# Aster32/GAN-DANet

Measured on AMD Instinct MI355X. Metric: train samples/sec (G+D step) on 256x256 tiles, higher is better.
Workload: dtype bf16; 1 GPU; full G+D train step, 8ch 256x256 -> 1024x1024 tiles, batch 32/GPU (global 32), perceptual=on, SSIM evaluated, AdamW x2; survey_config=3, per_gpu_batch=32, global_batch=32, tile=256, parallelism=dp1

## Files before the change

### gan-danet_amd/csrc/conv3x3.hip

```cpp
#include "common.h"
#include "tile_mma.h"
#include "../../include/gandanet.h"

namespace {

using gd::acc_row;
using gd::bf16x8_native_t;
typedef unsigned int u32x4_t __attribute__((ext_vector_type(4)));

constexpr int TW = 32;
constexpr int PW = TW + 2;
constexpr int CK = 32;
constexpr int LD = CK + 8;

__global__ void pack_w_kernel(const float* __restrict__ a, long a_sm, long a_sc, long a_st, int M, int Ck, int flip,
                              int BM, int nchunks, unsigned short* __restrict__ wp, long total) {
    for (long i = (long)blockIdx.x * blockDim.x + threadIdx.x; i < total; i += (long)gridDim.x * blockDim.x) {
        const int cc = (int)(i % CK);
        long t = i / CK;
        const int mm = (int)(t % BM);
        t /= BM;
        const int tap = (int)(t % 9);
        t /= 9;
        const int chunk = (int)(t % nchunks);
        const int mt = (int)(t / nchunks);
        const int m = mt * BM + mm, c = chunk * CK + cc;
        float v = 0.f;
        if (m < M && c < Ck) v = a[(long)m * a_sm + (long)c * a_sc + (long)(flip ? 8 - tap : tap) * a_st];
        wp[i] = gd_f2bf(v);
    }
}

template <int BM, int TH, int S>
__global__ __launch_bounds__(256, 2) void conv3x3_halo_kernel(const gd_conv_desc d, const unsigned short* __restrict__ wp,
                                                             int tiles_x, int nchunks) {
    constexpr int WAVES_M = 2, WAVES_N = 2;
    constexpr int TM = BM / (32 * WAVES_M);
    constexpr int TN = TH / WAVES_N;
    constexpr int PH = S * (TH - 1) + 3;
    constexpr int PWk = S * (TW - 1) + 3;
    constexpr int NPIX = PH * PWk;
    constexpr int WCHUNKS = 3 * BM * CK / 8;
    constexpr int WPT = WCHUNKS / 256;
    static_assert(WCHUNKS % 256 == 0, "weight stage must divide evenly");

    __shared__ __attribute__((aligned(16))) unsigned short patch[NPIX * LD];
    __shared__ __attribute__((aligned(16))) unsigned short wts[3 * BM * LD];

    const int tid = threadIdx.x, lane = tid & 63, wave = tid >> 6;
    const int r = lane & 31, h = lane >> 5;
    const int wm = wave >> 1, wn = wave & 1;
    const int b = blockIdx.z;
    const int mt = blockIdx.y;
    const int ty = blockIdx.x / tiles_x, tx = blockIdx.x - ty * tiles_x;
    const int y0 = ty * TH, x0 = tx * TW;
    const int H = d.Hi, W = d.Wi;
    const int Ho = d.Ho, Wo = d.Wo;
    const long HW = (long)H * W, HWo = (long)Ho * Wo;
    const float* ximg = d.x + (long)b * d.x_bs;

    f32x16_t acc[TM][TN];
#pragma unroll
    for (int i = 0; i < TM; ++i)
#pragma unroll
        for (int j = 0; j < TN; ++j)
#pragma unroll
            for (int e = 0; e < 16; ++e) acc[i][j][e] = 0.f;

    const unsigned short* wbase = wp + (long)mt * nchunks * 9 * BM * CK;
    u32x4_t wreg[WPT];
    auto load_w = [&](int chunk, int ky) {
        const u32x4_t* src = reinterpret_cast<const u32x4_t*>(wbase + ((long)chunk * 9 + ky * 3) * BM * CK);
#pragma unroll
        for (int i = 0; i < WPT; ++i) wreg[i] = src[tid + i * 256];
    };
    auto store_w = [&]() {
#pragma unroll
        for (int i = 0; i < WPT; ++i) {
            const int v = tid + i * 256;
            const int row = v >> 2, q = v & 3;
            *reinterpret_cast<u32x4_t*>(wts + row * LD + q * 8) = wreg[i];
        }
    };

    for (int chunk = 0; chunk < nchunks; ++chunk) {
        const int c0 = chunk * CK;
        load_w(chunk, 0);
        for (int w = tid; w < 2 * NPIX; w += 256) {
            const int half = w >= NPIX ? 1 : 0;
            const int pix = w - half * NPIX;
            const int py = pix / PWk, px = pix - py * PWk;
            const int iy = S * y0 - 1 + py, ix = S * x0 - 1 + px;
            const bool inside = iy >= 0 && iy < H && ix >= 0 && ix < W;
            const int cb = c0 + half * 16;
            const float* p = ximg + (long)cb * HW + (long)iy * W + ix;
            unsigned int* dst = reinterpret_cast<unsigned int*>(patch + pix * LD + half * 16);
#pragma unroll
            for (int j = 0; j < 8; ++j) {
                const int c = cb + 2 * j;
                float v0 = 0.f, v1 = 0.f;
                if (inside) {
                    if (c < d.Ck) v0 = p[(long)(2 * j) * HW];
                    if (c + 1 < d.Ck) v1 = p[(long)(2 * j + 1) * HW];
                    if (d.in_scale) {
                        if (c < d.Ck) {
                            v0 = fmaf(v0, d.in_scale[c], d.in_shift[c]);
                            if (d.in_relu) v0 = fmaxf(v0, 0.f);
                        }
                        if (c + 1 < d.Ck) {
                            v1 = fmaf(v1, d.in_scale[c + 1], d.in_shift[c + 1]);
                            if (d.in_relu) v1 = fmaxf(v1, 0.f);
                        }
                    }
                }
                dst[j] = gd_pack_bf2(v0, v1);
            }
        }
        for (int ky = 0; ky < 3; ++ky) {
            store_w();
            __syncthreads();
            if (ky < 2) load_w(chunk, ky + 1);
#pragma unroll
            for (int kx = 0; kx < 3; ++kx) {
#pragma unroll
                for (int ks = 0; ks < CK / 16; ++ks) {
                    bf16x8_t fa[TM], fb[TN];
#pragma unroll
                    for (int i = 0; i < TM; ++i)
                        fa[i] = *reinterpret_cast<const bf16x8_t*>(wts + (kx * BM + wm * TM * 32 + i * 32 + r) * LD +
                                                                  ks * 16 + 8 * h);
#pragma unroll
                    for (int j = 0; j < TN; ++j)
                        fb[j] = *reinterpret_cast<const bf16x8_t*>(patch + (((wn * TN + j) * S + ky) * PWk + r * S + kx) * LD +
                                                                  ks * 16 + 8 * h);
#pragma unroll
                    for (int i = 0; i < TM; ++i)
#pragma unroll
                        for (int j = 0; j < TN; ++j)
                            acc[i][j] = __builtin_amdgcn_mfma_f32_32x32x16_bf16(
                                __builtin_bit_cast(bf16x8_native_t, fa[i]), __builtin_bit_cast(bf16x8_native_t, fb[j]),
                                acc[i][j], 0, 0, 0);
                }
            }
            __syncthreads();
        }
    }

    const float alpha = d.alpha ? *d.alpha : 1.f;
    const int ox = x0 + r;
    if (ox < Wo) {
#pragma unroll
        for (int j = 0; j < TN; ++j) {
            const int oy = y0 + wn * TN + j;
            if (oy >= Ho) continue;
            const long pn = (long)oy * Wo + ox;
#pragma unroll
            for (int i = 0; i < TM; ++i)
#pragma unroll
                for (int e = 0; e < 16; ++e) {
                    const int m = mt * BM + wm * TM * 32 + i * 32 + acc_row(e, h);
                    if (m >= d.M) continue;
                    float v = acc[i][j][e] * alpha;
                    if (d.bias) v += d.bias[m];
                    if (d.res) v += d.res[(long)b * d.res_bs + (long)m * HWo + pn];
                    if (d.act == GD_ACT_RELU) v = fmaxf(v, 0.f);
                    else if (d.act == GD_ACT_LEAKY02) v = v >= 0.f ? v : 0.2f * v;
                    float* yp = reinterpret_cast<float*>(d.y) + (long)b * d.y_bs + (long)m * HWo + pn;
                    if (d.accumulate) v += *yp;
                    *yp = v;
                }
        }
    }
}

}

static inline int pick_bm(int M, int Ck) {
    if (Ck <= CK && M > 64) return 128;
    return (M <= 64 || (M % 128 != 0 && M % 128 <= 64)) ? 64 : 128;
}

extern "C" size_t gd_conv3x3_ws_bytes(int M, int Ck) {
    const int bm = pick_bm(M, Ck);
    const long mtiles = (M + bm - 1) / bm, nchunks = (Ck + CK - 1) / CK;
    return (size_t)(mtiles * bm * nchunks * CK * 9 * 2);
}

extern "C" int gd_conv3x3_eligible(const gd_conv_desc* d) {
    if (!(d && d->ks == 3 && d->pad == 1 && d->out_layout == 0 && !d->out_bf16 && d->precision == GD_PREC_BF16 &&
          d->a_bs == 0 && (d->Mstore == 0 || d->Mstore == d->M) && d->sub_step <= 1))
        return 0;
    if (d->stride == 1) return d->Hi == d->Ho && d->Wi == d->Wo;
    return d->stride == 2 && !d->transposed && (d->Hi - 1) / 2 + 1 == d->Ho && (d->Wi - 1) / 2 + 1 == d->Wo;
}

extern "C" int gd_conv3x3(const gd_conv_desc* dp, void* ws, size_t ws_bytes, void* stream) {
    GD_CHECK_ARG(dp && ws, "gd_conv3x3: null argument");
    GD_CHECK_ARG(gd_conv3x3_eligible(dp), "gd_conv3x3: descriptor not eligible (needs 3x3, pad 1, stride 1 or forward stride 2, bf16, fp32 NCHW out)");
    const gd_conv_desc& d = *dp;
    GD_CHECK_ARG(d.B > 0 && d.B <= 65535 && d.M > 0 && d.Ck > 0 && d.Hi > 0 && d.Wi > 0, "gd_conv3x3: bad sizes");
    GD_CHECK_ARG(d.a && d.x && d.y, "gd_conv3x3: null tensor");
    GD_CHECK_ARG((d.in_scale == nullptr) == (d.in_shift == nullptr), "gd_conv3x3: in_scale/in_shift must come together");
    GD_CHECK_ARG(ws_bytes >= gd_conv3x3_ws_bytes(d.M, d.Ck), "gd_conv3x3: workspace too small");
    hipStream_t s = (hipStream_t)stream;
    const int bm = pick_bm(d.M, d.Ck);
    const int mtiles = (d.M + bm - 1) / bm, nchunks = (d.Ck + CK - 1) / CK;
    const long total = (long)mtiles * nchunks * 9 * bm * CK;
    {
        int blocks = (int)((total + 255) / 256);
        if (blocks > 2048) blocks = 2048;
        hipLaunchKernelGGL(pack_w_kernel, dim3(blocks), dim3(256), 0, s, d.a, d.a_sm, d.a_sc, d.a_st, d.M, d.Ck,
                           d.transposed ? 1 : 0, bm, nchunks, (unsigned short*)ws, total);
    }
    const int th = d.stride == 1 ? 8 : 4;
    const int tiles_x = (d.Wo + TW - 1) / TW, tiles_y = (d.Ho + th - 1) / th;
    GD_CHECK_ARG((long)tiles_x * tiles_y < (1L << 31), "gd_conv3x3: image too large");
    dim3 grid(tiles_x * tiles_y, mtiles, d.B);
    const unsigned short* wpk = (const unsigned short*)ws;
    if (d.stride == 1) {
        if (bm == 64) hipLaunchKernelGGL((conv3x3_halo_kernel<64, 8, 1>), grid, dim3(256), 0, s, d, wpk, tiles_x, nchunks);
        else hipLaunchKernelGGL((conv3x3_halo_kernel<128, 8, 1>), grid, dim3(256), 0, s, d, wpk, tiles_x, nchunks);
    } else {
        if (bm == 64) hipLaunchKernelGGL((conv3x3_halo_kernel<64, 4, 2>), grid, dim3(256), 0, s, d, wpk, tiles_x, nchunks);
        else hipLaunchKernelGGL((conv3x3_halo_kernel<128, 4, 2>), grid, dim3(256), 0, s, d, wpk, tiles_x, nchunks);
    }
    GD_LAUNCH_CHECK();
    return 0;
}

namespace {

struct NhwcConvArgs {
    const unsigned short* x;
    const unsigned short* wp;
    const float* bias;
    const unsigned short* mask;
    const unsigned short* res;
    unsigned short* y;
    float* y32;
    long y32_bs;
    int H, W, Ho, Wo, K, M, act, tiles_x, nchunks;
    float slope;
    int osplit;
};

template <int BM, int S, int EPI = 0>
__global__ __launch_bounds__(256, 2) void conv3x3_nhwc_kernel(const NhwcConvArgs a) {
    constexpr int TH = S == 1 ? 8 : 4;
    constexpr int WAVES_M = 2, WAVES_N = 2;
    constexpr int TM = BM / (32 * WAVES_M);
    constexpr int TN = TH / WAVES_N;
    constexpr int PH = S * (TH - 1) + 3, PWk = S * (TW - 1) + 3, NPIX = PH * PWk;
    constexpr int WCHUNKS = 3 * BM * CK / 8;
    constexpr int WPT = WCHUNKS / 256;
    constexpr int NIT = (4 * NPIX + 255) / 256;
    static_assert(WCHUNKS % 256 == 0, "weight stage must divide evenly");

    __shared__ __attribute__((aligned(16))) unsigned short patch[NPIX * LD];
    __shared__ __attribute__((aligned(16))) unsigned short wts[3 * BM * LD];

    const int tid = threadIdx.x, lane = tid & 63, wave = tid >> 6;
    const int r = lane & 31, h = lane >> 5;
    const int wm = wave >> 1, wn = wave & 1;
    const int b = blockIdx.z, mt = blockIdx.y;
    const int ty = blockIdx.x / a.tiles_x, tx = blockIdx.x - ty * a.tiles_x;
    const int y0 = ty * TH, x0 = tx * TW;
    const int H = a.H, W = a.W, K = a.K;
    const unsigned short* ximg = a.x + (long)b * H * W * K;

    f32x16_t acc[TM][TN];
#pragma unroll
    for (int i = 0; i < TM; ++i)
#pragma unroll
        for (int j = 0; j < TN; ++j)
#pragma unroll
            for (int e = 0; e < 16; ++e) acc[i][j][e] = 0.f;

    const unsigned short* wbase = a.wp + (long)mt * a.nchunks * 9 * BM * CK;
    u32x4_t wreg[WPT];
    auto load_w = [&](int chunk, int ky) {
        const u32x4_t* src = reinterpret_cast<const u32x4_t*>(wbase + ((long)chunk * 9 + ky * 3) * BM * CK);
#pragma unroll
        for (int i = 0; i < WPT; ++i) wreg[i] = src[tid + i * 256];
    };
    auto store_w = [&]() {
#pragma unroll
        for (int i = 0; i < WPT; ++i) {
            const int v = tid + i * 256;
            const int row = v >> 2, q = v & 3;
            *reinterpret_cast<u32x4_t*>(wts + row * LD + q * 8) = wreg[i];
        }
    };

    unsigned int goff[NIT], inmask = 0, slotmask = 0;
    int loff[NIT];
#pragma unroll
    for (int it = 0; it < NIT; ++it) {
        const int w = tid + it * 256;
        const int pix = w >> 2, q = w & 3;
        const int py = pix / PWk, px = pix - py * PWk;
        const int iy = S * y0 - 1 + py, ix = S * x0 - 1 + px;
        const bool slot = w < 4 * NPIX;
        const bool inside = slot && iy >= 0 && iy < H && ix >= 0 && ix < W;
        loff[it] = pix * LD + q * 8;
        goff[it] = inside ? (unsigned int)(((long)iy * W + ix) * K + q * 8) : 0u;
        inmask |= inside ? (1u << it) : 0u;
        slotmask |= slot ? (1u << it) : 0u;
    }
    u32x4_t raw[NIT];
    auto load_patch = [&](int chunk) {
        const unsigned short* base = ximg + chunk * CK;
#pragma unroll
        for (int it = 0; it < NIT; ++it) {
            const int q = (tid + it * 256) & 3;
            const u32x4_t z = {0u, 0u, 0u, 0u};
            raw[it] = (((inmask >> it) & 1u) && chunk * CK + q * 8 < K) ? *reinterpret_cast<const u32x4_t*>(base + goff[it]) : z;
        }
    };
    auto store_patch = [&]() {
#pragma unroll
        for (int it = 0; it < NIT; ++it)
            if ((slotmask >> it) & 1u) *reinterpret_cast<u32x4_t*>(patch + loff[it]) = raw[it];
    };

    load_patch(0);
    store_patch();
    for (int chunk = 0; chunk < a.nchunks; ++chunk) {
        load_w(chunk, 0);
#pragma unroll
        for (int ky = 0; ky < 3; ++ky) {
            store_w();
            __syncthreads();
            if (ky == 0 && chunk + 1 < a.nchunks) load_patch(chunk + 1);
            if (ky < 2) load_w(chunk, ky + 1);
#pragma unroll
            for (int kx = 0; kx < 3; ++kx) {
#pragma unroll
                for (int ks = 0; ks < CK / 16; ++ks) {
                    bf16x8_t fa[TM], fb[TN];
#pragma unroll
                    for (int i = 0; i < TM; ++i)
                        fa[i] = *reinterpret_cast<const bf16x8_t*>(wts + (kx * BM + wm * TM * 32 + i * 32 + r) * LD +
                                                                  ks * 16 + 8 * h);
#pragma unroll
                    for (int j = 0; j < TN; ++j)
                        fb[j] = *reinterpret_cast<const bf16x8_t*>(patch + (((wn * TN + j) * S + ky) * PWk + r * S + kx) * LD +
                                                                  ks * 16 + 8 * h);
#pragma unroll
                    for (int i = 0; i < TM; ++i)
#pragma unroll
                        for (int j = 0; j < TN; ++j)
                            acc[i][j] = __builtin_amdgcn_mfma_f32_32x32x16_bf16(
                                __builtin_bit_cast(bf16x8_native_t, fa[i]), __builtin_bit_cast(bf16x8_native_t, fb[j]),
                                acc[i][j], 0, 0, 0);
                }
            }
            __syncthreads();
        }
        if (chunk + 1 < a.nchunks) store_patch();
    }

    if constexpr (EPI == 1) {
        constexpr int SLD = LD;
        static_assert(4 * 2 * 32 * SLD <= NPIX * LD, "per-wave scratch must fit in the patch image");
        unsigned short* scr = patch + wave * (2 * 32 * SLD);
        const int RS = a.osplit ? 3 * a.M : a.M;
        const int ox = x0 + r;
#pragma unroll
        for (int j = 0; j < TN; ++j) {
            const int oy = y0 + wn * TN + j;
            if (oy >= a.Ho) continue;
            const long prow = ((long)b * a.Ho + oy) * a.Wo;
#pragma unroll
            for (int i = 0; i < TM; ++i) {
                const int mbase = mt * BM + wm * TM * 32 + i * 32;
                if (mbase >= a.M) continue;
#pragma unroll
                for (int g = 0; g < 4; ++g) {
                    const int m = mbase + 8 * g + 4 * h;
                    const bool ok = ox < a.Wo && m < a.M;
                    float v[4];
#pragma unroll
                    for (int k = 0; k < 4; ++k) {
                        v[k] = acc[i][j][4 * g + k];
                        if (a.bias && ok) v[k] += a.bias[m + k];
                        if (a.act == 1) v[k] = fmaxf(v[k], 0.f);
                        else if (a.act == 2) v[k] = v[k] > 0.f ? v[k] : v[k] * a.slope;
                    }
                    if (ok) {
                        const long pbase = (prow + ox) * RS;
                        if (a.mask) {
                            const uint2 mk = *reinterpret_cast<const uint2*>(a.mask + pbase + m);
                            if (!((mk.x & 0x7FFFu) && !(mk.x & 0x8000u))) v[0] = 0.f;
                            if (!((mk.x >> 16) & 0x7FFFu) || (mk.x >> 31)) v[1] = 0.f;
                            if (!((mk.y & 0x7FFFu) && !(mk.y & 0x8000u))) v[2] = 0.f;
                            if (!((mk.y >> 16) & 0x7FFFu) || (mk.y >> 31)) v[3] = 0.f;
                        }
                        if (a.res) {
#pragma unroll
                            for (int part = 0; part < 2; ++part) {
                                if (part && !a.osplit) break;
                                const uint2 rr = *reinterpret_cast<const uint2*>(a.res + pbase + part * a.M + m);
                                v[0] += gd_bf2f((unsigned short)(rr.x & 0xFFFFu));
                                v[1] += gd_bf2f((unsigned short)(rr.x >> 16));
                                v[2] += gd_bf2f((unsigned short)(rr.y & 0xFFFFu));
                                v[3] += gd_bf2f((unsigned short)(rr.y >> 16));
                            }
                        }
                    }
                    uint2 hi, lo = make_uint2(0u, 0u);
                    if (a.osplit) {
                        gd_split_bf2(v[0], v[1], hi.x, lo.x);
                        gd_split_bf2(v[2], v[3], hi.y, lo.y);
                        *reinterpret_cast<uint2*>(scr + 32 * SLD + r * SLD + 8 * g + 4 * h) = lo;
                    } else {
                        hi.x = gd_pack_bf2(v[0], v[1]);
                        hi.y = gd_pack_bf2(v[2], v[3]);
                    }
                    *reinterpret_cast<uint2*>(scr + r * SLD + 8 * g + 4 * h) = hi;
                }
#pragma unroll
                for (int pass = 0; pass < 2; ++pass) {
                    const int px = pass * 16 + (lane >> 2), c8 = (lane & 3) * 8;
                    const int oxp = x0 + px, m = mbase + c8;
                    if (oxp < a.Wo && m < a.M) {
                        unsigned short* dst = a.y + (prow + oxp) * RS + m;
                        const u32x4_t vh = *reinterpret_cast<const u32x4_t*>(scr + px * SLD + c8);
                        *reinterpret_cast<u32x4_t*>(dst) = vh;
                        if (a.osplit) {
                            *reinterpret_cast<u32x4_t*>(dst + a.M) = *reinterpret_cast<const u32x4_t*>(scr + 32 * SLD + px * SLD + c8);
                            *reinterpret_cast<u32x4_t*>(dst + 2 * a.M) = vh;
                        }
                    }
                }
            }
        }
        return;
    }

    const int ox = x0 + r;
    if (ox < a.Wo) {
#pragma unroll
        for (int j = 0; j < TN; ++j) {
            const int oy = y0 + wn * TN + j;
            if (oy >= a.Ho) continue;
            const long pbase = (((long)b * a.Ho + oy) * a.Wo + ox) * (a.osplit ? 3 * a.M : a.M);
#pragma unroll
            for (int i = 0; i < TM; ++i)
#pragma unroll
                for (int g = 0; g < 4; ++g) {
                    const int m = mt * BM + wm * TM * 32 + i * 32 + 8 * g + 4 * h;
                    if (m >= a.M) continue;
                    float v[4];
#pragma unroll
                    for (int k = 0; k < 4; ++k) {
                        v[k] = acc[i][j][4 * g + k];
                        if (a.bias) v[k] += a.bias[m + k];
                        if (a.act == 1) v[k] = fmaxf(v[k], 0.f);
                        else if (a.act == 2) v[k] = v[k] > 0.f ? v[k] : v[k] * a.slope;
                    }
                    if (a.mask) {
                        const uint2 mk = *reinterpret_cast<const uint2*>(a.mask + pbase + m);
                        if (!((mk.x & 0x7FFFu) && !(mk.x & 0x8000u))) v[0] = 0.f;
                        if (!((mk.x >> 16) & 0x7FFFu) || (mk.x >> 31)) v[1] = 0.f;
                        if (!((mk.y & 0x7FFFu) && !(mk.y & 0x8000u))) v[2] = 0.f;
                        if (!((mk.y >> 16) & 0x7FFFu) || (mk.y >> 31)) v[3] = 0.f;
                    }
                    if (a.res) {
#pragma unroll
                        for (int part = 0; part < 2; ++part) {
                            if (part && !a.osplit) break;
                            const uint2 rr = *reinterpret_cast<const uint2*>(a.res + pbase + part * a.M + m);
                            v[0] += gd_bf2f((unsigned short)(rr.x & 0xFFFFu));
                            v[1] += gd_bf2f((unsigned short)(rr.x >> 16));
                            v[2] += gd_bf2f((unsigned short)(rr.y & 0xFFFFu));
                            v[3] += gd_bf2f((unsigned short)(rr.y >> 16));
                        }
                    }
                    float* yp = a.y32 + (long)b * a.y32_bs + (long)m * a.Ho * a.Wo + (long)oy * a.Wo + ox;
#pragma unroll
                    for (int k = 0; k < 4; ++k) yp[(long)k * a.Ho * a.Wo] = v[k];
                }
        }
    }
}

struct NhwcDgrad2Args {
    const unsigned short* dy;
    const unsigned short* wp;
    const unsigned short* act;
    unsigned short* dx;
    int H, W, Ho, Wo, K, M, tiles_x, nchunks;
    float slope;
    int split;
};

__global__ __launch_bounds__(256, 2) void conv3x3_nhwc_dgrad2_kernel(const NhwcDgrad2Args a) {
    constexpr int BM = 64, TH = 4;
    constexpr int TN = TH / 2;
    constexpr int PH = TH + 1, PWd = TW + 1, NPIX = PH * PWd;
    constexpr int WPT = 3 * BM * CK / 8 / 256;
    constexpr int NIT = (4 * NPIX + 255) / 256;

    __shared__ __attribute__((aligned(16))) unsigned short patch[NPIX * LD];
    __shared__ __attribute__((aligned(16))) unsigned short wts[3 * BM * LD];

    const int tid = threadIdx.x, lane = tid & 63, wave = tid >> 6;
    const int r = lane & 31, h = lane >> 5;
    const int wm = wave >> 1, wn = wave & 1;
    const int b = blockIdx.z, mt = blockIdx.y;
    const int ty = blockIdx.x / a.tiles_x, tx = blockIdx.x - ty * a.tiles_x;
    const int u0 = ty * TH, v0 = tx * TW;
    const int Ho = a.Ho, Wo = a.Wo, M = a.M;
    const unsigned short* dyimg = a.dy + (long)b * Ho * Wo * M;

    f32x16_t acc[4][TN];
#pragma unroll
    for (int c = 0; c < 4; ++c)
#pragma unroll
        for (int j = 0; j < TN; ++j)
#pragma unroll
            for (int e = 0; e < 16; ++e) acc[c][j][e] = 0.f;

    const unsigned short* wbase = a.wp + (long)mt * a.nchunks * 9 * BM * CK;
    u32x4_t wreg[WPT];
    auto load_w = [&](int chunk, int ky) {
        const u32x4_t* src = reinterpret_cast<const u32x4_t*>(wbase + ((long)chunk * 9 + ky * 3) * BM * CK);
#pragma unroll
        for (int i = 0; i < WPT; ++i) wreg[i] = src[tid + i * 256];
    };
    auto store_w = [&]() {
#pragma unroll
        for (int i = 0; i < WPT; ++i) {
            const int v = tid + i * 256;
            *reinterpret_cast<u32x4_t*>(wts + (v >> 2) * LD + (v & 3) * 8) = wreg[i];
        }
    };

    unsigned int goff[NIT], inmask = 0, slotmask = 0;
    int loff[NIT];
#pragma unroll
    for (int it = 0; it < NIT; ++it) {
        const int w = tid + it * 256;
        const int pix = w >> 2, q = w & 3;
        const int py = pix / PWd, px = pix - py * PWd;
        const int iy = u0 + py, ix = v0 + px;
        const bool slot = w < 4 * NPIX;
        const bool inside = slot && iy < Ho && ix < Wo;
        loff[it] = pix * LD + q * 8;
        goff[it] = inside ? (unsigned int)(((long)iy * Wo + ix) * M + q * 8) : 0u;
        inmask |= inside ? (1u << it) : 0u;
        slotmask |= slot ? (1u << it) : 0u;
    }
    u32x4_t raw[NIT];
    auto load_patch = [&](int chunk) {
        const unsigned short* base = dyimg + chunk * CK;
#pragma unroll
        for (int it = 0; it < NIT; ++it) {
            const int q = (tid + it * 256) & 3;
            const u32x4_t z = {0u, 0u, 0u, 0u};
            raw[it] = (((inmask >> it) & 1u) && chunk * CK + q * 8 < M) ? *reinterpret_cast<const u32x4_t*>(base + goff[it]) : z;
        }
    };
    auto store_patch = [&]() {
#pragma unroll
        for (int it = 0; it < NIT; ++it)
            if ((slotmask >> it) & 1u) *reinterpret_cast<u32x4_t*>(patch + loff[it]) = raw[it];
    };

    load_patch(0);
    store_patch();
    for (int chunk = 0; chunk < a.nchunks; ++chunk) {
        load_w(chunk, 0);
#pragma unroll
        for (int ky = 0; ky < 3; ++ky) {
            store_w();
            __syncthreads();
            if (ky == 0 && chunk + 1 < a.nchunks) load_patch(chunk + 1);
            if (ky < 2) load_w(chunk, ky + 1);
            const int py = (ky + 1) & 1, oy = ky == 0 ? 1 : 0;
#pragma unroll
            for (int kx = 0; kx < 3; ++kx) {
                const int px = (kx + 1) & 1, ox = kx == 0 ? 1 : 0;
#pragma unroll
                for (int ks = 0; ks < CK / 16; ++ks) {
                    const bf16x8_t fa = *reinterpret_cast<const bf16x8_t*>(wts + (kx * BM + wm * 32 + r) * LD + ks * 16 + 8 * h);
#pragma unroll
                    for (int j = 0; j < TN; ++j) {
                        const bf16x8_t fb = *reinterpret_cast<const bf16x8_t*>(
                            patch + ((wn * TN + j + oy) * PWd + r + ox) * LD + ks * 16 + 8 * h);
                        acc[2 * py + px][j] = __builtin_amdgcn_mfma_f32_32x32x16_bf16(
                            __builtin_bit_cast(bf16x8_native_t, fa), __builtin_bit_cast(bf16x8_native_t, fb),
                            acc[2 * py + px][j], 0, 0, 0);
                    }
                }
            }
            __syncthreads();
        }
        if (chunk + 1 < a.nchunks) store_patch();
    }

#pragma unroll
    for (int c = 0; c < 4; ++c) {
        const int py = c >> 1, px = c & 1;
        const int X = 2 * (v0 + r) + px;
        if (X >= a.W) continue;
#pragma unroll
        for (int j = 0; j < TN; ++j) {
            const int Y = 2 * (u0 + wn * TN + j) + py;
            if (Y >= a.H) continue;
            const long pbase = (((long)b * a.H + Y) * a.W + X) * (a.split ? 3 * a.K : a.K);
#pragma unroll
            for (int g = 0; g < 4; ++g) {
                const int m = mt * BM + wm * 32 + 8 * g + 4 * h;
                if (m >= a.K) continue;
                float v[4];
#pragma unroll
                for (int k = 0; k < 4; ++k) v[k] = acc[c][j][4 * g + k];
                if (a.act) {
                    const uint2 mk = *reinterpret_cast<const uint2*>(a.act + pbase + m);
                    if (!((mk.x & 0x7FFFu) && !(mk.x & 0x8000u))) v[0] *= a.slope;
                    if (!((mk.x >> 16) & 0x7FFFu) || (mk.x >> 31)) v[1] *= a.slope;
                    if (!((mk.y & 0x7FFFu) && !(mk.y & 0x8000u))) v[2] *= a.slope;
                    if (!((mk.y >> 16) & 0x7FFFu) || (mk.y >> 31)) v[3] *= a.slope;
                }
                uint2 o;
                if (a.split) {
                    uint2 lo;
                    gd_split_bf2(v[0], v[1], o.x, lo.x);
                    gd_split_bf2(v[2], v[3], o.y, lo.y);
                    *reinterpret_cast<uint2*>(a.dx + pbase + a.K + m) = lo;
                    *reinterpret_cast<uint2*>(a.dx + pbase + 2 * a.K + m) = o;
                } else {
                    o.x = gd_pack_bf2(v[0], v[1]);
                    o.y = gd_pack_bf2(v[2], v[3]);
                }
                *reinterpret_cast<uint2*>(a.dx + pbase + m) = o;
            }
        }
    }
}

}

extern "C" int gd_conv3x3_nhwc_pack(const float* w, int Cout, int Cin, int transposed, void* ws, size_t ws_bytes,
                                    void* stream) {
    GD_CHECK_ARG(w && ws && Cout > 0 && Cin > 0 && transposed >= 0 && transposed <= 2, "gd_conv3x3_nhwc_pack: bad arguments");
    const int M = transposed ? Cin : Cout, K = transposed ? Cout : Cin;
    GD_CHECK_ARG(ws_bytes >= gd_conv3x3_ws_bytes(M, K), "gd_conv3x3_nhwc_pack: workspace too small");
    const int bm = transposed == 2 ? 64 : pick_bm(M, K);
    const int mtiles = (M + bm - 1) / bm, nchunks = (K + CK - 1) / CK;
    const long total = (long)mtiles * nchunks * 9 * bm * CK;
    int blocks = (int)((total + 255) / 256);
    if (blocks > 2048) blocks = 2048;
    const long sm = transposed ? 9 : (long)Cin * 9, sc = transposed ? (long)Cin * 9 : 9;
    hipLaunchKernelGGL(pack_w_kernel, dim3(blocks), dim3(256), 0, (hipStream_t)stream, w, sm, sc, 1L, M, K,
                       transposed == 1 ? 1 : 0, bm, nchunks, (unsigned short*)ws, total);
    GD_LAUNCH_CHECK();
    return 0;
}

static int nhwc_conv_launch(const void* x, const void* wpack, const float* bias, const void* mask, const void* res,
                            void* y, int B, int H, int W, int K, int M, int stride, int act, float slope, void* stream,
                            float* y32 = nullptr, long y32_bs = 0, int osplit = 0) {
    NhwcConvArgs a;
    a.y32 = y32; a.y32_bs = y32_bs; a.osplit = osplit;
    a.x = (const unsigned short*)x; a.wp = (const unsigned short*)wpack; a.bias = bias;
    a.mask = (const unsigned short*)mask; a.res = (const unsigned short*)res; a.y = (unsigned short*)y;
    a.H = H; a.W = W; a.K = K; a.M = M; a.act = act; a.slope = slope;
    a.Ho = (H - 1) / stride + 1; a.Wo = (W - 1) / stride + 1;
    const int bm = pick_bm(M, K);
    const int mtiles = (M + bm - 1) / bm;
    a.nchunks = (K + CK - 1) / CK;
    a.tiles_x = (a.Wo + TW - 1) / TW;
    const int th = stride == 1 ? 8 : 4;
    const int tiles_y = (a.Ho + th - 1) / th;
    dim3 grid(a.tiles_x * tiles_y, mtiles, B);
    hipStream_t s = (hipStream_t)stream;
    if (!a.y32) {
        if (stride == 1) {
            if (bm == 64) hipLaunchKernelGGL((conv3x3_nhwc_kernel<64, 1, 1>), grid, dim3(256), 0, s, a);
            else hipLaunchKernelGGL((conv3x3_nhwc_kernel<128, 1, 1>), grid, dim3(256), 0, s, a);
        } else {
            if (bm == 64) hipLaunchKernelGGL((conv3x3_nhwc_kernel<64, 2, 1>), grid, dim3(256), 0, s, a);
            else hipLaunchKernelGGL((conv3x3_nhwc_kernel<128, 2, 1>), grid, dim3(256), 0, s, a);
        }
    } else if (stride == 1) {
        if (bm == 64) hipLaunchKernelGGL((conv3x3_nhwc_kernel<64, 1>), grid, dim3(256), 0, s, a);
        else hipLaunchKernelGGL((conv3x3_nhwc_kernel<128, 1>), grid, dim3(256), 0, s, a);
    } else {
        if (bm == 64) hipLaunchKernelGGL((conv3x3_nhwc_kernel<64, 2>), grid, dim3(256), 0, s, a);
        else hipLaunchKernelGGL((conv3x3_nhwc_kernel<128, 2>), grid, dim3(256), 0, s, a);
    }
    GD_LAUNCH_CHECK();
    return 0;
}

extern "C" int gd_conv3x3_nhwc(const void* x, const void* wpack, const float* bias, const void* mask, const void* res,
                               void* y, int B, int H, int W, int K, int M, int relu, int split, void* stream) {
    GD_CHECK_ARG(x && wpack && y, "gd_conv3x3_nhwc: null pointer");
    GD_CHECK_ARG(B > 0 && B <= 65535 && H > 0 && W > 0 && K > 0 && M > 0 && K % 8 == 0 && M % 8 == 0,
                 "gd_conv3x3_nhwc: channel counts must be multiples of 8");
    GD_CHECK_ARG((long)H * W * K < (1L << 31) && (long)H * W * M * (split ? 3 : 1) < (1L << 31), "gd_conv3x3_nhwc: image too large");
    return nhwc_conv_launch(x, wpack, bias, mask, res, y, B, H, W, K, M, 1, relu ? 1 : 0, 0.f, stream, nullptr, 0, split ? 1 : 0);
}

extern "C" int gd_conv3x3_nhwc_f32out(const void* x, const void* wpack, const float* bias, float* y32, long y_bs, int B, int H,
                                      int W, int K, int M, int relu, void* stream) {
    GD_CHECK_ARG(x && wpack && y32, "gd_conv3x3_nhwc_f32out: null pointer");
    GD_CHECK_ARG(B > 0 && B <= 65535 && H > 0 && W > 0 && K > 0 && M > 0 && K % 8 == 0 && M % 4 == 0 && y_bs >= (long)M * H * W,
                 "gd_conv3x3_nhwc_f32out: K must be a multiple of 8, M of 4");
    GD_CHECK_ARG((long)H * W * K < (1L << 31), "gd_conv3x3_nhwc_f32out: image too large");
    return nhwc_conv_launch(x, wpack, bias, nullptr, nullptr, nullptr, B, H, W, K, M, 1, relu ? 1 : 0, 0.f, stream, y32, y_bs);
}

extern "C" int gd_conv3x3_nhwc_s2(const void* x, const void* wpack, const float* bias, void* y, int B, int H, int W, int K,
                                  int M, int act, float slope, int split, void* stream) {
    GD_CHECK_ARG(x && wpack && y, "gd_conv3x3_nhwc_s2: null pointer");
    GD_CHECK_ARG(B > 0 && B <= 65535 && H > 0 && W > 0 && K > 0 && M > 0 && K % 8 == 0 && M % 8 == 0 && act >= 0 && act <= 2,
                 "gd_conv3x3_nhwc_s2: channel counts must be multiples of 8, act in 0..2");
    GD_CHECK_ARG((long)H * W * K < (1L << 31) && (long)H * W * M * (split ? 3 : 1) < (1L << 31), "gd_conv3x3_nhwc_s2: image too large");
    return nhwc_conv_launch(x, wpack, bias, nullptr, nullptr, y, B, H, W, K, M, 2, act, slope, stream, nullptr, 0, split ? 1 : 0);
}

extern "C" int gd_conv3x3_nhwc_s2_dgrad(const void* dy, const void* wpack_t, const void* act_out, float slope, void* dx,
                                        int B, int H, int W, int K, int M, int split, void* stream) {
    GD_CHECK_ARG(dy && wpack_t && dx, "gd_conv3x3_nhwc_s2_dgrad: null pointer");
    GD_CHECK_ARG(B > 0 && B <= 65535 && H > 0 && W > 0 && K > 0 && M > 0 && K % 8 == 0 && M % 8 == 0,
                 "gd_conv3x3_nhwc_s2_dgrad: channel counts must be multiples of 8");
    GD_CHECK_ARG((long)H * W * K * (split ? 3 : 1) < (1L << 31) && (long)H * W * M < (1L << 31), "gd_conv3x3_nhwc_s2_dgrad: image too large");
    NhwcDgrad2Args a;
    a.split = split ? 1 : 0;
    a.dy = (const unsigned short*)dy; a.wp = (const unsigned short*)wpack_t; a.act = (const unsigned short*)act_out;
    a.dx = (unsigned short*)dx; a.H = H; a.W = W; a.K = K; a.M = M; a.slope = slope;
    a.Ho = (H - 1) / 2 + 1; a.Wo = (W - 1) / 2 + 1;
    a.nchunks = (M + CK - 1) / CK;
    a.tiles_x = (a.Wo + TW - 1) / TW;
    const int tiles_y = (a.Ho + 3) / 4;
    dim3 grid(a.tiles_x * tiles_y, (K + 63) / 64, B);
    hipLaunchKernelGGL(conv3x3_nhwc_dgrad2_kernel, grid, dim3(256), 0, (hipStream_t)stream, a);
    GD_LAUNCH_CHECK();
    return 0;
}

namespace {

typedef short s16x4_t __attribute__((ext_vector_type(4)));
constexpr int WTH = 4;
constexpr int WPH = WTH + 2;
constexpr int WNPIX = WPH * PW;
constexpr int DYLD = WTH * TW + 8;

struct WgradArgs {
    const unsigned short* dy16;
    const float* dy; long dy_bs;
    const float* x; long x_bs;
    const unsigned short* x16; int x16_ld;
    const float* in_scale; const float* in_shift; int in_relu;
    float* dw;
    float* part;
    int B, M, Ck, H, W, Ho, Wo;
    int tiles_x, tiles_y, tiles_per_split;
};
typedef float f32x4u_t __attribute__((ext_vector_type(4), aligned(4)));

__device__ __forceinline__ s16x4_t lds_tr_read(const unsigned short* p) {
    return __builtin_amdgcn_ds_read_tr16_b64_v4i16((__attribute__((address_space(3))) s16x4_t*)p);
}

#ifndef GD_WGRAD_PIPED_MINW
#define GD_WGRAD_PIPED_MINW 1
#endif
template <int NW, int S, bool CS, bool PIPED = false, bool ORD = false>
__global__ __launch_bounds__(NW * 64, PIPED ? GD_WGRAD_PIPED_MINW : 2) void conv3x3_wgrad_kernel(const WgradArgs a) {
    constexpr int BM = CS ? 32 : 32 * NW, NT = 64 * NW, NCH = CS ? NW : 1;
    constexpr int PHk = S * (WTH - 1) + 3, PWk = S * (TW - 1) + 3, NPIXk = PHk * PWk;
    __shared__ __attribute__((aligned(16))) unsigned short dys[BM * DYLD];
    __shared__ __attribute__((aligned(16))) unsigned short patch[NCH * NPIXk * LD];

    const int tid = threadIdx.x, lane = tid & 63, wave = tid >> 6;
    const int r = lane & 31, h = lane >> 5;
    const int c0 = blockIdx.x * CK * NCH;
    const int m0 = blockIdx.y * BM;
    const long HW = (long)a.H * a.W;
    const long HWo = (long)a.Ho * a.Wo;
    const int ntiles = a.B * a.tiles_y * a.tiles_x;
    const int t_begin = blockIdx.z * a.tiles_per_split;
    const int t_end = min(ntiles, t_begin + a.tiles_per_split);

    f32x16_t acc[9];
#pragma unroll
    for (int t = 0; t < 9; ++t)
#pragma unroll
        for (int e = 0; e < 16; ++e) acc[t][e] = 0.f;

    const int li = lane & 15, tq = li >> 2, tp = li & 3, tg = (lane >> 4) & 1;
    const bool vec_ok = (a.Wo % 4) == 0;

    constexpr bool piped = PIPED;
    constexpr int NDY = PIPED ? (BM * 32 + NT - 1) / NT : 1;
    constexpr int NXI = PIPED ? (4 * NCH * NPIXk + NT - 1) / NT : 1;
    uint2 rdy[NDY];
    u32x4_t rxp[NXI];
    auto load_regs = [&](int t) {
        const int b = t / (a.tiles_y * a.tiles_x);
        const int rem = t - b * (a.tiles_y * a.tiles_x);
        const int ty_ = rem / a.tiles_x, tx_ = rem - ty_ * a.tiles_x;
        const int y0 = ty_ * WTH, x0 = tx_ * TW;
#pragma unroll
        for (int k = 0; k < NDY; ++k) {
            const int idx = tid + k * NT;
            const int m = idx >> 5, v = idx & 31;
            const int yy = y0 + (v >> 3), xx = x0 + (v & 7) * 4;
            uint2 w = make_uint2(0u, 0u);
            if (idx < BM * 32 && m0 + m < a.M && yy < a.Ho) {
                const unsigned short* p = a.dy16 + ((long)b * a.M + m0 + m) * HWo + (long)yy * a.Wo + xx;
                if (vec_ok && xx + 3 < a.Wo) {
                    w = *reinterpret_cast<const uint2*>(p);
                } else {
                    unsigned int e0 = xx + 0 < a.Wo ? p[0] : 0u, e1 = xx + 1 < a.Wo ? p[1] : 0u;
                    unsigned int e2 = xx + 2 < a.Wo ? p[2] : 0u, e3 = xx + 3 < a.Wo ? p[3] : 0u;
                    w.x = e0 | (e1 << 16);
                    w.y = e2 | (e3 << 16);
                }
            }
            rdy[k] = w;
        }
#pragma unroll
        for (int k = 0; k < NXI; ++k) {
            const int w = tid + k * NT;
            const int oc = w / NPIXk;
            const int q = oc & 3, chk = oc >> 2;
            const int pix = w - oc * NPIXk;
            const int py = pix / PWk, px = pix - py * PWk;
            const int iy = S * y0 - 1 + py, ix = S * x0 - 1 + px;
            const int cb = c0 + chk * CK + q * 8;
            u32x4_t v = {0u, 0u, 0u, 0u};
            if (w < 4 * NCH * NPIXk && iy >= 0 && iy < a.H && ix >= 0 && ix < a.W && cb < a.x16_ld)
                v = *reinterpret_cast<const u32x4_t*>(a.x16 + (((long)b * a.H + iy) * a.W + ix) * a.x16_ld + cb);
            rxp[k] = v;
        }
    };
    auto store_regs = [&]() {
#pragma unroll
        for (int k = 0; k < NDY; ++k) {
            const int idx = tid + k * NT;
            if (idx < BM * 32) *reinterpret_cast<uint2*>(dys + (idx >> 5) * DYLD + (idx & 31) * 4) = rdy[k];
        }
#pragma unroll
        for (int k = 0; k < NXI; ++k) {
            const int w = tid + k * NT;
            if (w < 4 * NCH * NPIXk) {
                const int oc = w / NPIXk;
                const int pix = w - oc * NPIXk;
                *reinterpret_cast<u32x4_t*>(patch + ((oc >> 2) * NPIXk + pix) * LD + (oc & 3) * 8) = rxp[k];
            }
        }
    };
    if constexpr (piped) {
        if (t_begin < t_end) load_regs(t_begin);
    }

    for (int t = t_begin; t < t_end; ++t) {
        const int b = t / (a.tiles_y * a.tiles_x);
        const int rem = t - b * (a.tiles_y * a.tiles_x);
        const int ty_ = rem / a.tiles_x, tx_ = rem - ty_ * a.tiles_x;
        const int y0 = ty_ * WTH, x0 = tx_ * TW;
        const float* dyb = a.dy + (long)b * a.dy_bs;
        const float* xb = a.x + (long)b * a.x_bs;

        if constexpr (piped) {
            store_regs();
        } else {
#pragma unroll 4
        for (int k = 0; k < 16 / (CS ? NW : 1) + (CS && (16 % NW) ? 1 : 0); ++k) {
            const int idx = tid + k * NT;
            if (CS && idx >= 32 * 32) break;
            const int m = idx >> 5, v = idx & 31;
            const int yy = y0 + (v >> 3), xx = x0 + (v & 7) * 4;
            if (a.dy16) {
                uint2 w = make_uint2(0u, 0u);
                if (m0 + m < a.M && yy < a.Ho) {
                    const unsigned short* p = a.dy16 + ((long)b * a.M + m0 + m) * HWo + (long)yy * a.Wo + xx;
                    if (vec_ok && xx + 3 < a.Wo) {
                        w = *reinterpret_cast<const uint2*>(p);
                    } else {
                        unsigned int e0 = xx + 0 < a.Wo ? p[0] : 0u, e1 = xx + 1 < a.Wo ? p[1] : 0u;
                        unsigned int e2 = xx + 2 < a.Wo ? p[2] : 0u, e3 = xx + 3 < a.Wo ? p[3] : 0u;
                        w.x = e0 | (e1 << 16);
                        w.y = e2 | (e3 << 16);
                    }
                }
                *reinterpret_cast<uint2*>(dys + m * DYLD + v * 4) = w;
                continue;
            }
            float4 f = make_float4(0.f, 0.f, 0.f, 0.f);
            if (m0 + m < a.M && yy < a.Ho) {
                const float* p = dyb + (long)(m0 + m) * HWo + (long)yy * a.Wo + xx;
                if (vec_ok && xx + 3 < a.Wo) {
                    f = *reinterpret_cast<const float4*>(p);
                } else {
                    if (xx + 0 < a.Wo) f.x = p[0];
// ... 232 lines not shown
```

Baseline: 38.17 samples/s.

## Swizzle LDS layout and double-buffer weight/patch stages in NHWC conv kernels

Replaces the padded LDS rows (LD=CK+8) with dense CK-wide rows and an XOR swizzle of 16-byte chunks, and de-interleaves stride-2 patch columns so strided reads avoid bank conflicts. Weight tiles are double-buffered in LDS when the footprint fits, which removes one __syncthreads per ky step. The transposed/upsample kernel also double-buffers the patch. This reduces barrier stalls and LDS padding, at the cost of more LDS per block, which may affect occupancy, and more intricate synchronization.

Result: no change. 38.24 samples/s, median of 6 (+0.2%).

```diff
diff --git a/gan-danet_amd/csrc/conv3x3.hip b/gan-danet_amd/csrc/conv3x3.hip
--- a/gan-danet_amd/csrc/conv3x3.hip
+++ b/gan-danet_amd/csrc/conv3x3.hip
@@ -230,6 +230,10 @@
 
 namespace {
 
+__device__ __forceinline__ int swz8(int key, int q) { return (q ^ ((key >> 2) & 3)) * 8; }
+
+constexpr int LDS_BLOCK_BYTES = 80 * 1024;
+
 struct NhwcConvArgs {
     const unsigned short* x;
     const unsigned short* wp;
@@ -255,9 +259,13 @@
     constexpr int WPT = WCHUNKS / 256;
     constexpr int NIT = (4 * NPIX + 255) / 256;
     static_assert(WCHUNKS % 256 == 0, "weight stage must divide evenly");
-
-    __shared__ __attribute__((aligned(16))) unsigned short patch[NPIX * LD];
-    __shared__ __attribute__((aligned(16))) unsigned short wts[3 * BM * LD];
+    constexpr int PIMG = NPIX * CK, WIMG = 3 * BM * CK;
+    constexpr bool DBW = 2 * (PIMG + 2 * WIMG) <= LDS_BLOCK_BYTES;
+    constexpr int PEVEN = (PWk + 1) / 2;
+    auto ppos = [](int px) { return S == 1 ? px : (px & 1) * PEVEN + (px >> 1); };
+
+    __shared__ __attribute__((aligned(16))) unsigned short patch[PIMG];
+    __shared__ __attribute__((aligned(16))) unsigned short wts[(DBW ? 2 : 1) * WIMG];
 
     const int tid = threadIdx.x, lane = tid & 63, wave = tid >> 6;
     const int r = lane & 31, h = lane >> 5;
@@ -283,12 +291,12 @@
 #pragma unroll
         for (int i = 0; i < WPT; ++i) wreg[i] = src[tid + i * 256];
     };
-    auto store_w = [&]() {
+    auto store_w = [&](unsigned short* wdst) {
 #pragma unroll
         for (int i = 0; i < WPT; ++i) {
             const int v = tid + i * 256;
             const int row = v >> 2, q = v & 3;
-            *reinterpret_cast<u32x4_t*>(wts + row * LD + q * 8) = wreg[i];
+            *reinterpret_cast<u32x4_t*>(wdst + row * CK + swz8(row, q)) = wreg[i];
         }
     };
 
@@ -302,7 +310,7 @@
         const int iy = S * y0 - 1 + py, ix = S * x0 - 1 + px;
         const bool slot = w < 4 * NPIX;
         const bool inside = slot && iy >= 0 && iy < H && ix >= 0 && ix < W;
-        loff[it] = pix * LD + q * 8;
+        loff[it] = (py * PWk + ppos(px)) * CK + swz8(ppos(px), q);
         goff[it] = inside ? (unsigned int)(((long)iy * W + ix) * K + q * 8) : 0u;
         inmask |= inside ? (1u << it) : 0u;
         slotmask |= slot ? (1u << it) : 0u;
@@ -317,52 +325,90 @@
             raw[it] = (((inmask >> it) & 1u) && chunk * CK + q * 8 < K) ? *reinterpret_cast<const u32x4_t*>(base + goff[it]) : z;
         }
     };
-    auto store_patch = [&]() {
+    auto store_patch = [&](unsigned short* pdst) {
 #pragma unroll
         for (int it = 0; it < NIT; ++it)
-            if ((slotmask >> it) & 1u) *reinterpret_cast<u32x4_t*>(patch + loff[it]) = raw[it];
+            if ((slotmask >> it) & 1u) *reinterpret_cast<u32x4_t*>(pdst + loff[it]) = raw[it];
+    };
+
+    int woff[CK / 16], poff[3][CK / 16];
+#pragma unroll
+    for (int ks = 0; ks < CK / 16; ++ks) {
+        woff[ks] = (wm * TM * 32 + r) * CK + swz8(r, 2 * ks + h);
+#pragma unroll
+        for (int kx = 0; kx < 3; ++kx) {
+            const int pos = ppos(r * S + kx);
+            poff[kx][ks] = (wn * TN * S * PWk + pos) * CK + swz8(pos, 2 * ks + h);
+        }
+    }
+    auto mma_row = [&](int ky, const unsigned short* wcur, const unsigned short* pcur) {
+#pragma unroll
+        for (int kx = 0; kx < 3; ++kx) {
+#pragma unroll
+            for (int ks = 0; ks < CK / 16; ++ks) {
+                bf16x8_t fa[TM], fb[TN];
+#pragma unroll
+                for (int i = 0; i < TM; ++i)
+                    fa[i] = *reinterpret_cast<const bf16x8_t*>(wcur + (kx * BM + i * 32) * CK + woff[ks]);
+#pragma unroll
+                for (int j = 0; j < TN; ++j)
+                    fb[j] = *reinterpret_cast<const bf16x8_t*>(pcur + (j * S + ky) * PWk * CK + poff[kx][ks]);
+#pragma unroll
+                for (int i = 0; i < TM; ++i)
+#pragma unroll
+                    for (int j = 0; j < TN; ++j)
+                        acc[i][j] = __builtin_amdgcn_mfma_f32_32x32x16_bf16(
+                            __builtin_bit_cast(bf16x8_native_t, fa[i]), __builtin_bit_cast(bf16x8_native_t, fb[j]),
+                            acc[i][j], 0, 0, 0);
+            }
+        }
     };
 
     load_patch(0);
-    store_patch();
-    for (int chunk = 0; chunk < a.nchunks; ++chunk) {
-        load_w(chunk, 0);
-#pragma unroll
-        for (int ky = 0; ky < 3; ++ky) {
-            store_w();
-            __syncthreads();
-            if (ky == 0 && chunk + 1 < a.nchunks) load_patch(chunk + 1);
-            if (ky < 2) load_w(chunk, ky + 1);
-#pragma unroll
-            for (int kx = 0; kx < 3; ++kx) {
-#pragma unroll
-                for (int ks = 0; ks < CK / 16; ++ks) {
-                    bf16x8_t fa[TM], fb[TN];
-#pragma unroll
-                    for (int i = 0; i < TM; ++i)
-                        fa[i] = *reinterpret_cast<const bf16x8_t*>(wts + (kx * BM + wm * TM * 32 + i * 32 + r) * LD +
-                                                                  ks * 16 + 8 * h);
-#pragma unroll
-                    for (int j = 0; j < TN; ++j)
-                        fb[j] = *reinterpret_cast<const bf16x8_t*>(patch + (((wn * TN + j) * S + ky) * PWk + r * S + kx) * LD +
-                                                                  ks * 16 + 8 * h);
-#pragma unroll
-                    for (int i = 0; i < TM; ++i)
-#pragma unroll
-                        for (int j = 0; j < TN; ++j)
-                            acc[i][j] = __builtin_amdgcn_mfma_f32_32x32x16_bf16(
-                                __builtin_bit_cast(bf16x8_native_t, fa[i]), __builtin_bit_cast(bf16x8_native_t, fb[j]),
-                                acc[i][j], 0, 0, 0);
-                }
-            }
-            __syncthreads();
-        }
-        if (chunk + 1 < a.nchunks) store_patch();
+    if constexpr (DBW) {
+        load_w(0, 0);
+        store_patch(patch);
+        store_w(wts);
+        load_w(0, 1);
+        int par = 0;
+        for (int chunk = 0; chunk < a.nchunks; ++chunk) {
+            const bool more = chunk + 1 < a.nchunks;
+#pragma unroll
+            for (int ky = 0; ky < 3; ++ky) {
+                __syncthreads();
+                if (ky < 2 || more) store_w(wts + (par ^ 1) * WIMG);
+                if (ky == 0) load_w(chunk, 2);
+                else if (more) load_w(chunk + 1, ky - 1);
+                if (ky == 0 && more) load_patch(chunk + 1);
+                mma_row(ky, wts + par * WIMG, patch);
+                par ^= 1;
+            }
+            if (more) {
+                __syncthreads();
+                store_patch(patch);
+            }
+        }
+        if constexpr (EPI == 1) __syncthreads();
+    } else {
+        store_patch(patch);
+        for (int chunk = 0; chunk < a.nchunks; ++chunk) {
+            load_w(chunk, 0);
+#pragma unroll
+            for (int ky = 0; ky < 3; ++ky) {
+                store_w(wts);
+                __syncthreads();
+                if (ky == 0 && chunk + 1 < a.nchunks) load_patch(chunk + 1);
+                if (ky < 2) load_w(chunk, ky + 1);
+                mma_row(ky, wts, patch);
+                __syncthreads();
+            }
+            if (chunk + 1 < a.nchunks) store_patch(patch);
+        }
     }
 
     if constexpr (EPI == 1) {
-        constexpr int SLD = LD;
-        static_assert(4 * 2 * 32 * SLD <= NPIX * LD, "per-wave scratch must fit in the patch image");
+        constexpr int SLD = CK + 8;
+        static_assert(4 * 2 * 32 * SLD <= PIMG, "per-wave scratch must fit in the patch image");
         unsigned short* scr = patch + wave * (2 * 32 * SLD);
         const int RS = a.osplit ? 3 * a.M : a.M;
         const int ox = x0 + r;
@@ -502,8 +548,10 @@
     constexpr int WPT = 3 * BM * CK / 8 / 256;
     constexpr int NIT = (4 * NPIX + 255) / 256;
 
-    __shared__ __attribute__((aligned(16))) unsigned short patch[NPIX * LD];
-    __shared__ __attribute__((aligned(16))) unsigned short wts[3 * BM * LD];
+    constexpr int PIMG = NPIX * CK, WIMG = 3 * BM * CK;
+    static_assert(2 * (2 * PIMG + 2 * WIMG) <= LDS_BLOCK_BYTES, "two blocks per CU");
+    __shared__ __attribute__((aligned(16))) unsigned short patch[2 * PIMG];
+    __shared__ __attribute__((aligned(16))) unsigned short wts[2 * WIMG];
 
     const int tid = threadIdx.x, lane = tid & 63, wave = tid >> 6;
     const int r = lane & 31, h = lane >> 5;
@@ -529,11 +577,11 @@
 #pragma unroll
         for (int i = 0; i < WPT; ++i) wreg[i] = src[tid + i * 256];
     };
-    auto store_w = [&]() {
+    auto store_w = [&](unsigned short* wdst) {
 #pragma unroll
         for (int i = 0; i < WPT; ++i) {
             const int v = tid + i * 256;
-            *reinterpret_cast<u32x4_t*>(wts + (v >> 2) * LD + (v & 3) * 8) = wreg[i];
+            *reinterpret_cast<u32x4_t*>(wdst + (v >> 2) * CK + swz8(v >> 2, v & 3)) = wreg[i];
         }
     };
 
@@ -547,7 +595,7 @@
         const int iy = u0 + py, ix = v0 + px;
         const bool slot = w < 4 * NPIX;
         const bool inside = slot && iy < Ho && ix < Wo;
-        loff[it] = pix * LD + q * 8;
+        loff[it] = pix * CK + swz8(px, q);
         goff[it] = inside ? (unsigned int)(((long)iy * Wo + ix) * M + q * 8) : 0u;
         inmask |= inside ? (1u << it) : 0u;
         slotmask |= slot ? (1u << it) : 0u;
@@ -562,42 +610,56 @@
             raw[it] = (((inmask >> it) & 1u) && chunk * CK + q * 8 < M) ? *reinterpret_cast<const u32x4_t*>(base + goff[it]) : z;
         }
     };
-    auto store_patch = [&]() {
+    auto store_patch = [&](unsigned short* pdst) {
 #pragma unroll
         for (int it = 0; it < NIT; ++it)
-            if ((slotmask >> it) & 1u) *reinterpret_cast<u32x4_t*>(patch + loff[it]) = raw[it];
-    };
+            if ((slotmask >> it) & 1u) *reinterpret_cast<u32x4_t*>(pdst + loff[it]) = raw[it];
+    };
+
+    int woff[CK / 16], poff[2][CK / 16];
+#pragma unroll
+    for (int ks = 0; ks < CK / 16; ++ks) {
+        woff[ks] = (wm * 32 + r) * CK + swz8(r, 2 * ks + h);
+#pragma unroll
+        for (int ox = 0; ox < 2; ++ox) poff[ox][ks] = (wn * TN * PWd + r + ox) * CK + swz8(r + ox, 2 * ks + h);
+    }
 
     load_patch(0);
-    store_patch();
+    load_w(0, 0);
+    store_patch(patch);
+    store_w(wts);
+    load_w(0, 1);
+    int par = 0;
     for (int chunk = 0; chunk < a.nchunks; ++chunk) {
-        load_w(chunk, 0);
+        const bool more = chunk + 1 < a.nchunks;
+        const unsigned short* pcur = patch + (chunk & 1) * PIMG;
 #pragma unroll
         for (int ky = 0; ky < 3; ++ky) {
-            store_w();
             __syncthreads();
-            if (ky == 0 && chunk + 1 < a.nchunks) load_patch(chunk + 1);
-            if (ky < 2) load_w(chunk, ky + 1);
+            if (ky < 2 || more) store_w(wts + (par ^ 1) * WIMG);
+            if (ky == 0) load_w(chunk, 2);
+            else if (more) load_w(chunk + 1, ky - 1);
+            if (ky == 0 && more) load_patch(chunk + 1);
+            const unsigned short* wcur = wts + par * WIMG;
             const int py = (ky + 1) & 1, oy = ky == 0 ? 1 : 0;
 #pragma unroll
             for (int kx = 0; kx < 3; ++kx) {
                 const int px = (kx + 1) & 1, ox = kx == 0 ? 1 : 0;
 #pragma unroll
                 for (int ks = 0; ks < CK / 16; ++ks) {
-                    const bf16x8_t fa = *reinterpret_cast<const bf16x8_t*>(wts + (kx * BM + wm * 32 + r) * LD + ks * 16 + 8 * h);
+                    const bf16x8_t fa = *reinterpret_cast<const bf16x8_t*>(wcur + kx * BM * CK + woff[ks]);
 #pragma unroll
                     for (int j = 0; j < TN; ++j) {
-                        const bf16x8_t fb = *reinterpret_cast<const bf16x8_t*>(
-                            patch + ((wn * TN + j + oy) * PWd + r + ox) * LD + ks * 16 + 8 * h);
+                        const bf16x8_t fb = *reinterpret_cast<const bf16x8_t*>(pcur + (j + oy) * PWd * CK + poff[ox][ks]);
                         acc[2 * py + px][j] = __builtin_amdgcn_mfma_f32_32x32x16_bf16(
                             __builtin_bit_cast(bf16x8_native_t, fa), __builtin_bit_cast(bf16x8_native_t, fb),
                             acc[2 * py + px][j], 0, 0, 0);
                     }
                 }
             }
-            __syncthreads();
-        }
-        if (chunk + 1 < a.nchunks) store_patch();
+            par ^= 1;
+        }
+        if (more) store_patch(patch + ((chunk + 1) & 1) * PIMG);
     }
 
 #pragma unroll
```
